# ubuntuslave/vo_single_camera_sos

Hardware: AMD Instinct MI355X
Metric: frame-pairs/sec (detect+match+triangulate+RANSAC) on 640x480 omni, 2000 kpts (higher is better)
Workload: dtype u8/f32/f64

## Files before the change

### vo_single_camera_sos_amd/csrc/ransac.hip

```cpp
#include <type_traits>
#include "common.h"
#include "ransac_core.h"
#include "epnp_core.h"
#include "gp3p_core.h"

namespace {

constexpr int kMaxCam = 8;
constexpr int kHypDoubles = 16;
constexpr int kThreads = 256;
constexpr int kScoreHypChunkMax = 128;

__device__ const double kEye9[9] = {1, 0, 0, 0, 1, 0, 0, 0, 1};
__device__ const double kZero3[3] = {0, 0, 0};

__device__ __forceinline__ uint64_t problem_seed(uint64_t seed, int b) { return seed + (uint64_t)b; }
__device__ __forceinline__ uint64_t problem_seed(const uint64_t* seeds, int b) { return seeds[b]; }

__global__ __launch_bounds__(kThreads) void ransac_prepare_kernel(const int32_t* __restrict__ cam,
                                                                  const int32_t* __restrict__ n_arr, int stride,
                                                                  int ncam, int32_t* __restrict__ perm,
                                                                  int32_t* __restrict__ cinfo,
                                                                  int32_t* __restrict__ split_out) {
  SOSVO_LATENCY_BOUND_PRIO();
// ... 137 lines not shown
                                                             const double* __restrict__ cam_off,
                                                             const double* __restrict__ cam_rot,
                                                             const int32_t* __restrict__ n_arr, int nprob, int stride,
                                                             int H, SeedT seed, double* __restrict__ hyp,
                                                             int32_t* __restrict__ counts) {
  SOSVO_LATENCY_BOUND_PRIO();
  int b, chunk;
  if (!hyp_block(nprob, (H + 63) >> 6, &b, &chunk)) return;
  const int it = chunk * 64 + threadIdx.x;
  const int n = min(n_arr[b], stride);
  const size_t base = (size_t)b * stride;
  const double* off = cam ? cam_off : kZero3;
  const double* rot = cam ? cam_rot : kEye9;
  double R[9], t[3];
  int ok = 0;
  if (it < H)
    ok = sv_hypothesis_gp3p(f + 3 * base, p + 3 * base, cam ? cam + base : nullptr, off, rot, n, problem_seed(seed, b),
                            (uint64_t)it, R, t);
  hyp_store_wave(hyp + (size_t)b * H * kHypDoubles, chunk * 64, H, ok != 0, R, t);
  if (it < H) counts[(size_t)b * H + it] = ok ? 0 : -1;
}

__device__ __forceinline__ int epnp_sample_front(const double* __restrict__ f, const double* __restrict__ p, int n, size_t base,
                                                 uint64_t seed, int it, double (&p6)[18], double (&uv)[2 * SV_EPNP_MAXN],
                                                 double (&cw)[12], double (&alphas)[4 * SV_EPNP_MAXN]) {
  int32_t s6[6];
  if (!sv_sample_distinct(n, 6, seed, (uint64_t)it, s6)) return 0;
  double f6[18];
#pragma unroll
  for (int k = 0; k < 6; ++k)
#pragma unroll
    for (int c = 0; c < 3; ++c) {
      f6[3 * k + c] = f[3 * (base + s6[k]) + c];
      p6[3 * k + c] = p[3 * (base + s6[k]) + c];
    }
  return sv_epnp_front(f6, p6, 6, uv, cw, alphas);
}

constexpr int kEpnpVecDoubles = 48;
template <class SeedT>
__global__ __launch_bounds__(64) void ransac_epnp_eigen_kernel(const double* __restrict__ f, const double* __restrict__ p,
                                                               const int32_t* __restrict__ n_arr, int nprob, int stride,
                                                               int H, SeedT seed, double* __restrict__ vvbuf,
                                                               int32_t* __restrict__ counts) {
  int b, chunk;
  if (!hyp_block(nprob, (H + 63) >> 6, &b, &chunk)) return;
  const int it = chunk * 64 + threadIdx.x;
  if (it >= H) return;
  const int n = min(n_arr[b], stride);
  double p6[18], uv[2 * SV_EPNP_MAXN], cw[12], alphas[4 * SV_EPNP_MAXN];
  int ok = epnp_sample_front(f, p, n, (size_t)b * stride, problem_seed(seed, b), it, p6, uv, cw, alphas);
  double* out = vvbuf + ((size_t)b * H + it) * kEpnpVecDoubles;
  if (ok) {
    double vv[48];
    ok = sv_epnp_null4_ql(alphas, uv, 6, vv);
    if (ok) {
#pragma unroll
      for (int k = 0; k < 48; ++k) out[k] = vv[k];
    }
  }
  counts[(size_t)b * H + it] = ok ? 0 : -1;
}

template <class SeedT>
__global__ __launch_bounds__(64) void ransac_epnp_pose_kernel(const double* __restrict__ f, const double* __restrict__ p,
                                                              const int32_t* __restrict__ n_arr, int nprob, int stride,
                                                              int H, SeedT seed, const double* __restrict__ vvbuf,
                                                              double* __restrict__ hyp, int32_t* __restrict__ counts) {
  SOSVO_LATENCY_BOUND_PRIO();
  int b, chunk;
  if (!hyp_block(nprob, (H + 63) >> 6, &b, &chunk)) return;
  const int it = chunk * 64 + threadIdx.x;
  const int n = min(n_arr[b], stride);
  double R[9], t[3];
  int ok = it < H && counts[(size_t)b * H + it] == 0;
  if (ok) {
    double p6[18], uv[2 * SV_EPNP_MAXN], cw[12], alphas[4 * SV_EPNP_MAXN], vv[48];
    ok = epnp_sample_front(f, p, n, (size_t)b * stride, problem_seed(seed, b), it, p6, uv, cw, alphas);
    const double* in = vvbuf + ((size_t)b * H + it) * kEpnpVecDoubles;
#pragma unroll
    for (int k = 0; k < 48; ++k) vv[k] = in[k];
    if (ok) ok = sv_epnp_back(p6, 6, uv, cw, alphas, vv, R, t);
  }
  hyp_store_wave(hyp + (size_t)b * H * kHypDoubles, chunk * 64, H, ok != 0, R, t);
  if (it < H) counts[(size_t)b * H + it] = ok ? 0 : -1;
}

template <bool IDENT>
__device__ __forceinline__ bool inlier_exact(const double* __restrict__ h, const double fx, const double fy,
                                             const double fz, const double px, const double py, const double pz,
                                             const double ox, const double oy, const double oz, const double* Rc,
                                             const double thr) {
  const double vx = (((h[0] * px) + (h[3] * py)) + (h[6] * pz)) + h[12];
  const double vy = (((h[1] * px) + (h[4] * py)) + (h[7] * pz)) + h[13];
  const double vz = (((h[2] * px) + (h[5] * py)) + (h[8] * pz)) + h[14];
  const double wx = vx - ox, wy = vy - oy, wz = vz - oz;
  double ux = wx, uy = wy, uz = wz;
  if (!IDENT) {
    ux = ((Rc[0] * wx) + (Rc[3] * wy)) + (Rc[6] * wz);
    uy = ((Rc[1] * wx) + (Rc[4] * wy)) + (Rc[7] * wz);
    uz = ((Rc[2] * wx) + (Rc[5] * wy)) + (Rc[8] * wz);
  }
  const double nrm = sqrt(((ux * ux) + (uy * uy)) + (uz * uz));
  const double gx = ux / nrm, gy = uy / nrm, gz = uz / nrm;
  return (1.0 - (((fx * gx) + (fy * gy)) + (fz * gz))) < thr;
}

constexpr double kTier1K = 1048576.0;
constexpr double kTier1Eps = 5.9604644775390625e-08;
constexpr double kTier1QBand = 3.47 / kTier1K + 20.0 * kTier1Eps;
constexpr double kTier1Max = 1e9;
constexpr double kTier1E2 = (3.47 * kTier1K + 6.0) * 78.03 * kTier1Eps * kTier1Eps * (1.0 + 1e-4);

__device__ __forceinline__ float score_tier1_lane(double fx, double fy, double fz, double px, double py, double pz, double ox,
                                                  double oy, double oz) {
  const double p1 = fabs(px) + fabs(py) + fabs(pz);
  const double om = fmax(fabs(ox), fmax(fabs(oy), fabs(oz)));
  const double fn = fx * fx + fy * fy + fz * fz;
  const double l = (p1 * p1 + om * om) * (1.0 + 1e-6);
  return (fabs(fn - 1.0) <= 1e-6 && p1 <= kTier1Max && om <= kTier1Max) ? (float)l : __builtin_inff();
}

__device__ __forceinline__ void score_tier1_hyp(const double* __restrict__ h, float* __restrict__ hs) {
  double rho = 0.0;
#pragma unroll
  for (int k = 0; k < 9; ++k) {
    hs[k] = (float)h[k];
    rho = fmax(rho, fabs(h[k]));
  }
  const double im = fmax(fabs(h[9]), fmax(fabs(h[10]), fabs(h[11])));
  hs[9] = (float)h[9], hs[10] = (float)h[10], hs[11] = (float)h[11];
  const double chk = (((((((h[0] + h[1]) + h[2]) + h[3]) + h[4]) + h[5]) + h[6]) + h[7]) + h[8] + h[9] + h[10] + h[11];
  const double ea = kTier1E2 * fmax(rho * rho, 1.0) * (1.0 + 1e-6);
  const double eb = kTier1E2 * (im * im) * (1.0 + 1e-6) + 1e-24;
  const bool fin = chk == chk && rho <= kTier1Max && im <= kTier1Max;
  hs[12] = fin ? (float)ea : __builtin_nanf("");
  hs[13] = fin ? (float)eb : __builtin_nanf("");
  hs[14] = 0.0f, hs[15] = 0.0f;
}

__device__ __forceinline__ int score_set_at(int E, int n, int split, int k) {
  if (split <= 0 || split >= n) return E - 1 - k;
  const int tb = split >> 6, nbot = E - 1 - tb, ntop = tb + 1, m = min(nbot, ntop);
  if (k < 2 * m) return (k & 1) ? tb - (k >> 1) : E - 1 - (k >> 1);
  return nbot > ntop ? E - 1 - (k - m) : tb - (k - m);
}

template <bool IDENT, int PPT, bool T1>
__global__ __launch_bounds__(kThreads) __attribute__((amdgpu_waves_per_eu(T1 ? 4 : 1))) void ransac_score_kernel(
    const double* __restrict__ f, const double* __restrict__ p, const int32_t* __restrict__ cam,
    const double* __restrict__ cam_off, const double* __restrict__ cam_rot, const int32_t* __restrict__ n_arr,
    int stride, int H, int hchunk, int hspan, double thr, int fast_ok, const double* __restrict__ hyp,
    int32_t* __restrict__ counts, int set_lo, int set_hi, int hsplit, const int32_t* __restrict__ alive_idx,
    const int32_t* __restrict__ n_alive, const int32_t* __restrict__ split_arr) {
  static_assert(!T1 || (IDENT && PPT <= 4), "tier 1 is written for the identity-rotation form");
  SOSVO_LATENCY_BOUND_PRIO();
  constexpr bool KEEP = !T1;
  __shared__ int lcnt[kScoreHypChunkMax];
  __shared__ double shyp[kScoreHypChunkMax][12];
  __shared__ unsigned long long sok[(kScoreHypChunkMax + 63) / 64];
  __shared__ int sidx[kScoreHypChunkMax];
  __shared__ int srec[kScoreHypChunkMax];
  __shared__ float shyp32[T1 ? kScoreHypChunkMax : 1][16];
  const int tid = threadIdx.x, b = blockIdx.z;
  const int n = min(n_arr[b], stride);
  const int Hb = alive_idx ? n_alive[b] : H;
  const int xspan = alive_idx ? (int)((blockIdx.x + blockIdx.z) % gridDim.x) : (int)blockIdx.x;
  if (xspan * hspan >= Hb) return;
  const int nset_all = (n + 63) >> 6, split = split_arr ? split_arr[b] : 0;
  auto set_at = [&](int k) { return split_arr ? score_set_at(nset_all, n, split, k) : k; };
  const int sbeg = set_lo, send = min(nset_all, set_hi);
  const int nsets = send - sbeg;
  const int bcap = hsplit ? PPT : (kThreads / 64) * PPT;
  const int nb = (nsets + bcap - 1) / bcap;
  if ((int)blockIdx.y >= nb) return;
  const int spb = (nsets + nb - 1) / nb;
  const int set0 = hsplit ? sbeg + ((int)blockIdx.y * nsets) / nb : sbeg + (int)blockIdx.y * spb;
  const int set1 = hsplit ? sbeg + (((int)blockIdx.y + 1) * nsets) / nb : min(set0 + spb, send);
  const int p0 = set_at(set0) * 64;

  double fx[KEEP ? PPT : 1], fy[KEEP ? PPT : 1], fz[KEEP ? PPT : 1];
  double px[KEEP ? PPT : 1], py[KEEP ? PPT : 1], pz[KEEP ? PPT : 1];
  double ox[KEEP ? PPT : 1], oy[KEEP ? PPT : 1], oz[KEEP ? PPT : 1];
  float fxs[T1 ? PPT : 1], fys[T1 ? PPT : 1], fzs[T1 ? PPT : 1], pxs[T1 ? PPT : 1], pys[T1 ? PPT : 1], pzs[T1 ? PPT : 1];
  float oxs[T1 ? PPT : 1], oys[T1 ? PPT : 1], ozs[T1 ? PPT : 1], lerr[T1 ? PPT : 1];
  int rowi[PPT];
  double Rc[IDENT ? 1 : 9];
  const int wave = __builtin_amdgcn_readfirstlane(tid >> 6), lane = tid & 63;
  const int wslot = (wave + blockIdx.x + blockIdx.y + blockIdx.z) & (kThreads / 64 - 1);
  const int jstep = hsplit ? kThreads / 64 : 1, jbeg = hsplit ? wslot : 0;
  const size_t base = (size_t)b * stride;
  unsigned long long vmask[PPT];
  int nlive_v = 0;
#pragma unroll
  for (int r = 0; r < PPT; ++r) {
    const int pos = set0 + (hsplit ? r : r * (kThreads / 64) + wslot);
    const int i0 = (pos < set1 ? set_at(pos) : nset_all) * 64;
    const int i = i0 + lane;
    nlive_v += pos < set1 ? 1 : 0;
    const bool valid = i < n;
    vmask[r] = __ballot(valid);
    rowi[r] = valid ? i : p0;
    const size_t row = base + rowi[r];
    const double lfx = f[3 * row + 0], lfy = f[3 * row + 1], lfz = f[3 * row + 2];
    const double lpx = p[3 * row + 0], lpy = p[3 * row + 1], lpz = p[3 * row + 2];
    const int c = cam ? cam[row] : 0;
    const double* o = cam ? cam_off + 3 * c : kZero3;
    const double lox = o[0], loy = o[1], loz = o[2];
    if (KEEP) {
      fx[r] = lfx, fy[r] = lfy, fz[r] = lfz;
      px[r] = lpx, py[r] = lpy, pz[r] = lpz;
      ox[r] = lox, oy[r] = loy, oz[r] = loz;
    }
    if (!IDENT) {
      const double* rc = cam ? cam_rot + 9 * c : kEye9;
#pragma unroll
      for (int k = 0; k < 9; ++k) Rc[k] = rc[k];
    }
    if (T1) {
      fxs[r] = (float)lfx, fys[r] = (float)lfy, fzs[r] = (float)lfz;
      pxs[r] = (float)lpx, pys[r] = (float)lpy, pzs[r] = (float)lpz;
      oxs[r] = (float)lox, oys[r] = (float)loy, ozs[r] = (float)loz;
      lerr[r] = score_tier1_lane(lfx, lfy, lfz, lpx, lpy, lpz, lox, loy, loz);
    }
  }
  const int nlive = __builtin_amdgcn_readfirstlane(nlive_v);
  const double c1 = 1.0 - thr;
  const double c2 = c1 * c1;
  const double c2hi = c2 * (1.0 + 1e-9), c2lo = c2 * (1.0 - 1e-9);
  const float c2hs = (float)((c2 + kTier1QBand) * (1.0 + 1e-6)), c2ls = (float)((c2 - kTier1QBand) * (1.0 - 1e-6));
  const int hend = min(Hb, (xspan + 1) * hspan);
  for (int h0 = xspan * hspan; h0 < hend; h0 += hchunk) {
  const int h1 = min(hend, h0 + hchunk);
  for (int k = tid; k < kScoreHypChunkMax; k += kThreads) lcnt[k] = 0;
  const int nh = h1 - h0;
  const double* hb = hyp + (size_t)b * H * kHypDoubles;
  static_assert(kScoreHypChunkMax == 128, "two words of solved-hypothesis flags");
  if (wave < 2) {
    const int hh = wave * 64 + lane;
    const int rec = hh < nh ? (alive_idx ? alive_idx[(size_t)b * H + h0 + hh] : h0 + hh) : 0;
    const double r00 = hh < nh ? hb[(size_t)rec * kHypDoubles] : 0.0;
    const unsigned long long okb = __ballot(hh < nh && r00 == r00);
    if (lane == 0) sok[wave] = okb;
    srec[hh] = rec;
  }
  __syncthreads();
  const unsigned long long ok0 = sok[0], ok1 = sok[1];
  const int nok = __builtin_amdgcn_readfirstlane(__popcll(ok0) + __popcll(ok1));
  for (int k = tid; k < nh * 12; k += kThreads) {
    const int hh = k / 12, e = k - hh * 12;
    const unsigned long long w = hh < 64 ? ok0 : ok1;
    if ((w >> (hh & 63)) & 1ULL) {
      const int pos = __popcll(w & ((1ULL << (hh & 63)) - 1ULL)) + (hh < 64 ? 0 : __popcll(ok0));
      const int rec = srec[hh];
      shyp[pos][e] = hb[(size_t)rec * kHypDoubles + (e < 9 ? e : e + 3)];
      if (e == 0) sidx[pos] = rec;
    }
  }
  __syncthreads();
  if (T1) {
    for (int pos = tid; pos < nok; pos += kThreads) score_tier1_hyp(shyp[pos], shyp32[pos]);
    __syncthreads();
  }

  auto tier2 = [&](auto nl, const int j, const unsigned long long* und1) -> int {
    constexpr int NL = decltype(nl)::value;
    int total = 0;
    const double* hp = shyp[j];
    const double r0 = hp[0], r1 = hp[1], r2 = hp[2], r3 = hp[3], r4 = hp[4], r5 = hp[5], r6 = hp[6], r7 = hp[7], r8 = hp[8];
    const double ix = hp[9], iy = hp[10], iz = hp[11];
#pragma unroll
    for (int r = 0; r < NL && r < PPT; ++r) {
      if (!und1[r]) continue;
      double Fx, Fy, Fz, Px, Py, Pz, Ox, Oy, Oz;
      if (KEEP) {
        Fx = fx[r], Fy = fy[r], Fz = fz[r], Px = px[r], Py = py[r], Pz = pz[r];
        Ox = ox[r], Oy = oy[r], Oz = oz[r];
      } else {
        const size_t row = base + rowi[r];
        Fx = f[3 * row + 0], Fy = f[3 * row + 1], Fz = f[3 * row + 2];
        Px = p[3 * row + 0], Py = p[3 * row + 1], Pz = p[3 * row + 2];
        const double* o = cam ? cam_off + 3 * cam[row] : kZero3;
        Ox = o[0], Oy = o[1], Oz = o[2];
      }
      unsigned long long und = und1[r];
      if (fast_ok) {
        double ux = fma(r0, Px, fma(r3, Py, fma(r6, Pz, ix - Ox)));
        double uy = fma(r1, Px, fma(r4, Py, fma(r7, Pz, iy - Oy)));
        double uz = fma(r2, Px, fma(r5, Py, fma(r8, Pz, iz - Oz)));
        if (!IDENT) {
          const double wx = ux, wy = uy, wz = uz;
          ux = fma(Rc[0], wx, fma(Rc[IDENT ? 0 : 3], wy, Rc[IDENT ? 0 : 6] * wz));
          uy = fma(Rc[IDENT ? 0 : 1], wx, fma(Rc[IDENT ? 0 : 4], wy, Rc[IDENT ? 0 : 7] * wz));
          uz = fma(Rc[IDENT ? 0 : 2], wx, fma(Rc[IDENT ? 0 : 5], wy, Rc[IDENT ? 0 : 8] * wz));
        }
        const double s = fma(Fx, ux, fma(Fy, uy, Fz * uz));
        const double q = fma(ux, ux, fma(uy, uy, uz * uz));
        const double lhs = s * s;
        const unsigned long long pos = __ballot(s > 0.0) & und1[r];
        const unsigned long long hi = __ballot(lhs > c2hi * q);
        const unsigned long long lo = __ballot(lhs < c2lo * q);
        total += __popcll(pos & hi);
        und = pos & ~hi & ~lo;
      }
      if (und) {
        const double vx = (((r0 * Px) + (r3 * Py)) + (r6 * Pz)) + ix;
        const double vy = (((r1 * Px) + (r4 * Py)) + (r7 * Pz)) + iy;
        const double vz = (((r2 * Px) + (r5 * Py)) + (r8 * Pz)) + iz;
        const double wx = vx - Ox, wy = vy - Oy, wz = vz - Oz;
        double ux = wx, uy = wy, uz = wz;
        if (!IDENT) {
          ux = ((Rc[0] * wx) + (Rc[IDENT ? 0 : 3] * wy)) + (Rc[IDENT ? 0 : 6] * wz);
          uy = ((Rc[IDENT ? 0 : 1] * wx) + (Rc[IDENT ? 0 : 4] * wy)) + (Rc[IDENT ? 0 : 7] * wz);
          uz = ((Rc[IDENT ? 0 : 2] * wx) + (Rc[IDENT ? 0 : 5] * wy)) + (Rc[IDENT ? 0 : 8] * wz);
        }
        const double q = ((ux * ux) + (uy * uy)) + (uz * uz);
        const double nrm = sqrt(q);
        const double gx = ux / nrm, gy = uy / nrm, gz = uz / nrm;
        total += __popcll(__ballot((1.0 - (((Fx * gx) + (Fy * gy)) + (Fz * gz))) < thr) & und);
      }
    }
    return total;
  };

  auto tier1 = [&](auto nl, const int j, unsigned long long* und1, unsigned long long& any1) -> int {
    constexpr int NL = decltype(nl)::value;
    int total = 0;
    const float* hs = shyp32[T1 ? j : 0];
    const float q0 = hs[0], q1 = hs[1], q2 = hs[2], q3 = hs[3], q4 = hs[4], q5 = hs[5], q6 = hs[6], q7 = hs[7], q8 = hs[8];
    const float jx = hs[9], jy = hs[10], jz = hs[11], ea = hs[12], eb = hs[13];
#pragma unroll
    for (int r = 0; r < NL && r < PPT; ++r) {
      const float ux = fmaf(q0, pxs[T1 ? r : 0], fmaf(q3, pys[T1 ? r : 0], fmaf(q6, pzs[T1 ? r : 0], jx - oxs[T1 ? r : 0])));
      const float uy = fmaf(q1, pxs[T1 ? r : 0], fmaf(q4, pys[T1 ? r : 0], fmaf(q7, pzs[T1 ? r : 0], jy - oys[T1 ? r : 0])));
      const float uz = fmaf(q2, pxs[T1 ? r : 0], fmaf(q5, pys[T1 ? r : 0], fmaf(q8, pzs[T1 ? r : 0], jz - ozs[T1 ? r : 0])));
      const float sv = fmaf(fxs[T1 ? r : 0], ux, fmaf(fys[T1 ? r : 0], uy, fzs[T1 ? r : 0] * uz));
      const float qv = fmaf(ux, ux, fmaf(uy, uy, uz * uz));
      const float lhs = sv * fabsf(sv);
      const float e2 = fmaf(ea, lerr[T1 ? r : 0], eb);
      const unsigned long long hi = __ballot(lhs > fmaf(c2hs, qv, e2));
      const unsigned long long lo = __ballot(lhs < fmaf(c2ls, qv, -e2));
      total += __popcll(hi & vmask[r]);
      und1[r] = ~hi & ~lo & vmask[r];
      any1 |= und1[r];
    }
    return total;
  };

  auto hyp_loop = [&](auto nl) {
    constexpr int NL = decltype(nl)::value;
    int cntv = 0, k = 0;
    for (int j = jbeg; j < nok; j += jstep, ++k) {
      unsigned long long und[PPT], any = 0ULL;
      int tot = 0;
      if (T1) {
        tot = tier1(nl, j, und, any);
      } else {
#pragma unroll
        for (int r = 0; r < NL && r < PPT; ++r) {
          und[r] = vmask[r];
          any |= vmask[r];
        }
      }
      if (any) tot += tier2(nl, j, und);
      if (lane == (k & 63)) cntv += tot;
      if ((k & 63) == 63) {
        if (cntv) atomicAdd(&lcnt[jbeg + ((k & ~63) + lane) * jstep], cntv);
        cntv = 0;
      }
    }
    if (cntv) atomicAdd(&lcnt[jbeg + (((k - 1) & ~63) + lane) * jstep], cntv);
  };
  if (nlive >= 4) hyp_loop(std::integral_constant<int, 4>{});
  else if (nlive == 3) hyp_loop(std::integral_constant<int, 3>{});
  else if (nlive == 2) hyp_loop(std::integral_constant<int, 2>{});
  else if (nlive == 1) hyp_loop(std::integral_constant<int, 1>{});
  __syncthreads();
  for (int k = tid; k < nok; k += kThreads) {
    const int v = lcnt[k];
    if (v) atomicAdd(&counts[(size_t)b * H + sidx[k]], v);
  }
  }
}

__global__ __launch_bounds__(kThreads) void ransac_prune_kernel(
    const double* __restrict__ f, const double* __restrict__ p, const int32_t* __restrict__ cam,
    const double* __restrict__ cam_off, const int32_t* __restrict__ n_arr, int stride, int H, int k_done, double thr,
    const double* __restrict__ hyp, const int32_t* __restrict__ counts, const int32_t* __restrict__ in_idx,
    const int32_t* __restrict__ n_in, int32_t* __restrict__ alive_idx, int32_t* __restrict__ n_alive,
    int32_t* __restrict__ state) {
  SOSVO_LATENCY_BOUND_PRIO();
  __shared__ long long red[kThreads / 64];
  __shared__ int redc[kThreads / 64];
  __shared__ int wave_off[kThreads / 64 + 1];
  const int tid = threadIdx.x, b = blockIdx.x, lane = tid & 63, wid = tid >> 6;
  const int n = min(n_arr[b], stride);
  const int32_t* cb = counts + (size_t)b * H;
  const int32_t* ib = in_idx ? in_idx + (size_t)b * H : nullptr;
  int32_t* ab = alive_idx + (size_t)b * H;
  const int Hin = in_idx ? n_in[b] : H;
  long long best_key = -1;
  for (int j = tid; j < Hin; j += kThreads) {
    const int it = ib ? ib[j] : j;
    const int c = cb[it];
    const long long key = ((long long)c << 32) | (long long)(0x7FFFFFFF - it);
    if (c >= 0 && key > best_key) best_key = key;
  }
  for (int o = 32; o > 0; o >>= 1) {
    const long long other = __shfl_down(best_key, o);
    best_key = other > best_key ? other : best_key;
  }
  if (lane == 0) red[wid] = best_key;
  __syncthreads();
  best_key = red[0];
  for (int w = 1; w < kThreads / 64; ++w) best_key = red[w] > best_key ? red[w] : best_key;
  if (best_key < 0) {
    if (tid == 0) n_alive[b] = 0;
    return;
  }
  const int hstar = 0x7FFFFFFF - (int)(best_key & 0xFFFFFFFFLL);
  const int L_prev = in_idx ? state[2 * b] : 0, h_prev = in_idx ? state[2 * b + 1] : -1;
  int L = L_prev;
  if (hstar != h_prev) {
    const double* hp = hyp + ((size_t)b * H + hstar) * kHypDoubles;
    const size_t base = (size_t)b * stride;
    int cnt = 0;
    for (int i = tid; i < n; i += kThreads) {
      const size_t row = base + i;
      const double* o = cam ? cam_off + 3 * cam[row] : kZero3;
      cnt += inlier_exact<true>(hp, f[3 * row], f[3 * row + 1], f[3 * row + 2], p[3 * row], p[3 * row + 1], p[3 * row + 2],
                                o[0], o[1], o[2], kEye9, thr) ? 1 : 0;
    }
    for (int o = 32; o > 0; o >>= 1) cnt += __shfl_down(cnt, o);
    if (lane == 0) redc[wid] = cnt;
    __syncthreads();
    L = max(L_prev, ((redc[0] + redc[1]) + redc[2]) + redc[3]);
  }
  const int rest = 64 * max(0, ((n + 63) >> 6) - k_done);
  int running = 0;
  for (int j0 = 0; j0 < Hin; j0 += kThreads) {
    const int j = j0 + tid;
    const int it = j < Hin ? (ib ? ib[j] : j) : 0;
    const int c = j < Hin ? cb[it] : -1;
    const bool keep = c >= 0 && c + rest >= L;
    const unsigned long long bal = __ballot(keep);
    __syncthreads();
    if (lane == 0) wave_off[wid + 1] = __popcll(bal);
    __syncthreads();
    int off = running;
    for (int w = 0; w < wid; ++w) off += wave_off[w + 1];
    if (keep) ab[off + __popcll(bal & ((1ULL << lane) - 1ULL))] = it;
    running += ((wave_off[1] + wave_off[2]) + wave_off[3]) + wave_off[4];
  }
  if (tid == 0) {
    n_alive[b] = running;
    state[2 * b] = L;
    state[2 * b + 1] = hstar;
  }
}

template <bool IDENT>
__global__ __launch_bounds__(kThreads) void ransac_select_kernel(
    const double* __restrict__ f, const double* __restrict__ p, const int32_t* __restrict__ cam,
    const double* __restrict__ cam_off, const double* __restrict__ cam_rot, const int32_t* __restrict__ n_arr,
    int stride, int H, double thr, int adaptive, const double* __restrict__ hyp, const int32_t* __restrict__ counts,
    double* __restrict__ T_out, uint8_t* __restrict__ mask, int32_t* __restrict__ inl_idx,
    int32_t* __restrict__ n_inl, int32_t* __restrict__ info) {
  SOSVO_LATENCY_BOUND_PRIO();
  __shared__ long long red[kThreads / 64];
  __shared__ int redv[kThreads / 64];
  __shared__ int s_best_it, s_used, s_nvalid;
  __shared__ int wave_off[kThreads / 64 + 1];
  __shared__ int s_running;
  const int tid = threadIdx.x, b = blockIdx.x, lane = tid & 63, wid = tid >> 6;
  const int n = min(n_arr[b], stride);
  const int32_t* cb = counts + (size_t)b * H;

  long long best_key = -1;
  int nvalid = 0;
  for (int it = tid; it < H; it += kThreads) {
    const int c = cb[it];
    if (c >= 0) {
      nvalid++;
      const long long key = ((long long)c << 32) | (long long)(0x7FFFFFFF - it);
      best_key = key > best_key ? key : best_key;
    }
  }
  for (int o = 32; o > 0; o >>= 1) {
    const long long other = __shfl_down(best_key, o);
    best_key = other > best_key ? other : best_key;
    nvalid += __shfl_down(nvalid, o);
  }
  if (lane == 0) {
    red[wid] = best_key;
    redv[wid] = nvalid;
  }
  __syncthreads();
  if (tid == 0) {
    long long k = red[0];
    int nv = redv[0];
    for (int w = 1; w < kThreads / 64; ++w) {
      k = red[w] > k ? red[w] : k;
      nv += redv[w];
    }
    s_nvalid = nv;
    if (!(adaptive & 1)) {
      s_best_it = k < 0 ? -1 : (0x7FFFFFFF - (int)(k & 0xFFFFFFFFLL));
      s_used = H;
    } else {
      int best_count = -1, best_it = -1, iterations = 0, used = 0;
      double base = 1.0;
      for (int it = 0; it < H; ++it) {
        if (iterations > 0 && !sv_ransac_continue(base, iterations)) break;
        used = it + 1;
        const int c = cb[it];
        if (c < 0) continue;
        if (c > best_count) {
          best_count = c;
          best_it = it;
          base = (adaptive & 2) ? sv_adaptive_base6(c, n) : ((adaptive & 4) ? sv_adaptive_base2(c, n) : sv_adaptive_base(c, n));
        }
        iterations++;
      }
      s_best_it = best_it;
      s_used = used;
    }
    s_running = 0;
  }
  __syncthreads();
  const int best_it = s_best_it;
  const size_t base = (size_t)b * stride;
  if (best_it < 0) {
    for (int i = tid; i < n; i += kThreads) mask[base + i] = 0;
// ... 161 lines not shown
        __syncthreads();
        continue;
      }
      if (s_flag == 4) {
        converged = 1;
        __syncthreads();
        break;
      }
      double xn[6];
#pragma unroll
      for (int u = 0; u < 6; ++u) xn[u] = sxn[u];
      double cn = 0.0;
      for (int q = tid; q < cnt; q += kThreads) {
        const int i = idx ? idx[base + q] : q;
        const size_t row = base + i;
        const int cc = cam ? cam[row] : 0;
        const double* o = cam ? cam_off + 3 * cc : kZero3;
        const double* rc = cam ? cam_rot + 9 * cc : kEye9;
        const double r = sv_residual(xn, f + 3 * row, p + 3 * row, o, rc);
        cn += r * r;
      }
      cn = block_sum(cn, scratch, tid);
      if (cn < cost) {
        converged = ((cost - cn) <= SV_LM_FTOL * cost);
        __syncthreads();
        if (tid == 0) {
#pragma unroll
          for (int u = 0; u < 6; ++u) sx[u] = xn[u];
        }
        cost = cn;
        lambda *= 0.1;
        if (lambda < 1e-15) lambda = 1e-15;
        accepted = 1;
        __syncthreads();
        break;
      }
      lambda *= 10.0;
      __syncthreads();
    }
    it_done = it + 1;
    if (!accepted || converged) break;
  }
  __syncthreads();
  if (tid == 0) {
    double R[9], t[3];
    sv_cayley2rot(sx + 3, R);
    t[0] = sx[0];
    t[1] = sx[1];
    t[2] = sx[2];
    sv_Rt_to_T(R, t, T);
    if (cost_out) cost_out[b] = cost;
    if (iters_out) iters_out[b] = it_done;
  }
}

}

template <class SeedT>
static int32_t ransac_abs_pose_impl(sosvo_ctx* ctx, const char* fn, const double* f, const double* p, const int32_t* cam,
                                    const double* cam_off, const double* cam_rot, int32_t ncam, int32_t flags,
                                    const int32_t* n, int32_t nprob, int32_t stride, double thr, int32_t max_iter,
                                    int32_t adaptive, SeedT seed, double* T_out,
                                    uint8_t* inlier_mask, int32_t* inlier_idx, int32_t* n_inliers, int32_t* info,
                                    int32_t* hyp_counts) {
#define SOSVO_LAUNCH_HYP(ctx, kernel, ...)              \
  do {                                                  \
    SOSVO_PROFILE(ctx, #kernel);                        \
    hipLaunchKernelGGL((kernel<SeedT>), __VA_ARGS__);   \
  } while (0)
#define SOSVO_REQUIRE_FN(ctx, cond, msg)                               \
  do {                                                                 \
    if (!(cond)) return sosvo_fail((ctx), SOSVO_ERR_ARG, fn, msg);     \
  } while (0)
  SOSVO_REQUIRE_FN(ctx, f && p && n && T_out && inlier_mask && inlier_idx && n_inliers && info, "null pointer");
  SOSVO_REQUIRE_FN(ctx, cam == nullptr || (cam_off && cam_rot), "cam given without cam_off / cam_rot");
  SOSVO_REQUIRE_FN(ctx, ncam >= 1 && ncam <= kMaxCam, "ncam out of range (1..8)");
  SOSVO_REQUIRE_FN(ctx, nprob >= 0 && nprob <= 65535, "nprob out of range");
  SOSVO_REQUIRE_FN(ctx, stride > 0 && stride <= (1 << 20), "stride out of range");
  SOSVO_REQUIRE_FN(ctx, max_iter > 0 && max_iter <= (1 << 20), "max_iter out of range");
  SOSVO_REQUIRE_FN(ctx, thr > 0.0, "threshold must be positive");
  if (nprob == 0) return SOSVO_OK;
  const int H = max_iter;
  size_t off = 0;
  auto carve = [&](size_t bytes) {
    size_t o = off;
    off += (bytes + 255) & ~(size_t)255;
    return o;
  };
  const size_t o_perm = carve(sizeof(int32_t) * (size_t)nprob * stride);
  const size_t o_cinfo = carve(sizeof(int32_t) * (size_t)nprob * (2 * kMaxCam + 1));
  const size_t o_hyp = carve(sizeof(double) * (size_t)nprob * H * kHypDoubles);
  const size_t o_counts = carve(sizeof(int32_t) * (size_t)nprob * H);
  const bool epnp_vec = (flags & SOSVO_FLAG_EPNP) != 0;
  const size_t o_vv = carve(epnp_vec ? sizeof(double) * (size_t)nprob * H * kEpnpVecDoubles : 0);
  const size_t o_alive = carve(sizeof(int32_t) * (size_t)nprob * (H + 1));
  const size_t o_alive2 = carve(sizeof(int32_t) * (size_t)nprob * (H + 1));
  const size_t o_stage = carve(sizeof(int32_t) * (size_t)nprob * 2);
  const size_t o_split = carve(sizeof(int32_t) * (size_t)nprob);
  int32_t rc = sosvo_ws_reserve(ctx, off);
  if (rc != SOSVO_OK) return rc;
  char* ws = (char*)ctx->ws;
  int32_t* perm = (int32_t*)(ws + o_perm);
  int32_t* cinfo = (int32_t*)(ws + o_cinfo);
  double* hyp = (double*)(ws + o_hyp);
  int32_t* counts = hyp_counts ? hyp_counts : (int32_t*)(ws + o_counts);
  int32_t* split = (int32_t*)(ws + o_split);

  SOSVO_LAUNCH(ctx,ransac_prepare_kernel, dim3(nprob), dim3(kThreads), 0, ctx->stream, cam, n, stride,
                     cam ? ncam : 1, perm, cinfo, split);
  SOSVO_LAUNCH_CHECK(ctx);
  const int epnp = (flags & SOSVO_FLAG_EPNP) != 0;
  SOSVO_REQUIRE_FN(ctx, !epnp || cam == nullptr, "SOSVO_FLAG_EPNP is for central problems (cam == NULL)");
  const int twopt = (flags & SOSVO_FLAG_TWOPT) != 0 && !epnp && !(flags & SOSVO_FLAG_GP3P);
  SOSVO_REQUIRE_FN(ctx, !twopt || cam == nullptr, "SOSVO_FLAG_TWOPT is for central problems (cam == NULL)");
  if (epnp) adaptive = (adaptive ? 1 : 0) | 2;
  if (twopt) adaptive = (adaptive ? 1 : 0) | 4;
  if (epnp) {
    double* vvbuf = (double*)(ws + o_vv);
    SOSVO_LAUNCH_HYP(ctx, ransac_epnp_eigen_kernel, dim3(hyp_grid(nprob, cdiv(H, 64))), dim3(64), 0, ctx->stream, f, p, n, nprob, stride, H,
                 seed, vvbuf, counts);
    SOSVO_LAUNCH_HYP(ctx, ransac_epnp_pose_kernel, dim3(hyp_grid(nprob, cdiv(H, 64))), dim3(64), 0, ctx->stream, f, p, n, nprob, stride, H,
                 seed, vvbuf, hyp, counts);
  } else if (twopt) {
    SOSVO_LAUNCH_HYP(ctx, ransac_hyp_twopt_kernel, dim3(hyp_grid(nprob, cdiv(H, 64))), dim3(64), 0, ctx->stream, f, p, n, nprob, stride, H, seed,
                 hyp, counts);
  } else if (flags & SOSVO_FLAG_GP3P) {
    SOSVO_LAUNCH_HYP(ctx, ransac_hyp_gp3p_kernel, dim3(hyp_grid(nprob, cdiv(H, 64))), dim3(64), 0, ctx->stream, f, p, cam, cam_off, cam_rot,
                 n, nprob, stride, H, seed, hyp, counts);
  } else
    SOSVO_LAUNCH_HYP(ctx, ransac_hyp_kernel, dim3(hyp_grid(nprob, cdiv(H, 64))), dim3(64), 0, ctx->stream, f, p, cam, cam_off, cam_rot, n,
                 nprob, stride, H, seed, perm, cinfo, hyp, counts);
  SOSVO_LAUNCH_CHECK(ctx);

  const bool ident = (flags & SOSVO_FLAG_CAM_ROT_IDENTITY) != 0 || cam == nullptr;
  const int fast_ok = thr < 0.5 ? 1 : 0;
  const int ppt = ident ? 4 : 1;
  const int gx = cdiv(stride, kThreads * ppt);
  const bool t1 = ident && fast_ok && !ctx->hint_score_fp64_only;
  const int wg_target = t1 ? 4096 : 8192;
  int hchunks = cdiv(wg_target, nprob);
  if (hchunks < 1) hchunks = 1;
  int hspan = cdiv(H, hchunks);
  if (hspan < 32) hspan = H < 32 ? H : 32;
  hchunks = cdiv(H, hspan);
  const int hchunk = cdiv(hspan, cdiv(hspan, kScoreHypChunkMax));
  dim3 grid(hchunks, gx, nprob);
  constexpr int kProbeSets = 4, kPruneMinSets = 8, kStageMinSets = 16, kPruneMinProblems = 64;
#ifndef SOSVO_STAGE_PLAN
#define SOSVO_STAGE_PLAN 4, 14
#endif
  static const int kStagePlan[] = {SOSVO_STAGE_PLAN};
  const bool prune = t1 && adaptive == 0 && hyp_counts == nullptr && !epnp && !twopt && stride >= 64 * kPruneMinSets &&
                     nprob >= kPruneMinProblems;
#define SOSVO_SCORE_ARGS grid, dim3(kThreads), 0, ctx->stream, f, p, cam, cam_off, cam_rot, n, stride, H, hchunk, hspan, thr, fast_ok, hyp, counts, 0, INT_MAX, 0, (const int32_t*)nullptr, (const int32_t*)nullptr, (const int32_t*)nullptr
  if (prune) {
    const int capsets = cdiv(stride, 64);
    const bool staged = stride >= 64 * kStageMinSets;
    int nstage = 1;
    if (staged)
      for (nstage = 0; nstage < (int)(sizeof(kStagePlan) / sizeof(kStagePlan[0])) && kStagePlan[nstage] < capsets;) ++nstage;
    int32_t* alive_idx[2] = {(int32_t*)(ws + o_alive), (int32_t*)(ws + o_alive2)};
    int32_t* stage_state = (int32_t*)(ws + o_stage);
    auto pass = [&](int k_lo, int k_hi, const int32_t* list) {
      const int sets = min(k_hi, capsets) - k_lo;
      int hs = min(H, (sets <= 4 ? 4 : 2) * hspan);
      if (list) hs = min(H, max(kScoreHypChunkMax, hs));
      const int hck = cdiv(hs, cdiv(hs, kScoreHypChunkMax));
      SOSVO_LAUNCH(ctx,(ransac_score_kernel<true, 4, true>), dim3(cdiv(H, hs), cdiv(sets, 4), nprob), dim3(kThreads), 0,
                   ctx->stream, f, p, cam, cam_off, cam_rot, n, stride, H, hck, hs, thr, fast_ok, hyp, counts, k_lo, k_hi, 1,
                   list, list ? list + (size_t)nprob * H : nullptr, split);
    };
    int k_lo = 0;
    const int32_t* list = nullptr;
    for (int s = 0; s < nstage; ++s) {
      const int k_hi = staged ? kStagePlan[s] : kProbeSets;
      pass(k_lo, k_hi, list);
      int32_t* out = alive_idx[s & 1];
      SOSVO_LAUNCH(ctx,ransac_prune_kernel, dim3(nprob), dim3(kThreads), 0, ctx->stream, f, p, cam, cam_off, n, stride, H,
                   k_hi, thr, hyp, counts, list, list ? list + (size_t)nprob * H : nullptr, out, out + (size_t)nprob * H,
                   stage_state);
      list = out;
      k_lo = k_hi;
    }
    pass(k_lo, INT_MAX, list);
  } else if (t1)
    SOSVO_LAUNCH(ctx,(ransac_score_kernel<true, 4, true>), SOSVO_SCORE_ARGS);
  else if (ident)
    SOSVO_LAUNCH(ctx,(ransac_score_kernel<true, 4, false>), SOSVO_SCORE_ARGS);
  else
    SOSVO_LAUNCH(ctx,(ransac_score_kernel<false, 1, false>), SOSVO_SCORE_ARGS);
#undef SOSVO_SCORE_ARGS
  SOSVO_LAUNCH_CHECK(ctx);
  if (ident)
    SOSVO_LAUNCH(ctx,(ransac_select_kernel<true>), dim3(nprob), dim3(kThreads), 0, ctx->stream, f, p, cam,
                       cam_off, cam_rot, n, stride, H, thr, adaptive, hyp, counts, T_out, inlier_mask, inlier_idx,
                       n_inliers, info);
  else
    SOSVO_LAUNCH(ctx,(ransac_select_kernel<false>), dim3(nprob), dim3(kThreads), 0, ctx->stream, f, p, cam,
                       cam_off, cam_rot, n, stride, H, thr, adaptive, hyp, counts, T_out, inlier_mask, inlier_idx,
                       n_inliers, info);
  SOSVO_LAUNCH_CHECK(ctx);
  return SOSVO_OK;
}
#undef SOSVO_REQUIRE_FN
#undef SOSVO_LAUNCH_HYP

extern "C" {

int32_t sosvo_ransac_abs_pose(sosvo_ctx* ctx, const double* f, const double* p, const int32_t* cam,
                              const double* cam_off, const double* cam_rot, int32_t ncam, int32_t flags,
                              const int32_t* n, int32_t nprob, int32_t stride, double thr, int32_t max_iter,
                              int32_t adaptive, uint64_t seed, double* T_out, uint8_t* inlier_mask,
                              int32_t* inlier_idx, int32_t* n_inliers, int32_t* info, int32_t* hyp_counts) {
  SOSVO_ENTER(ctx);
  return ransac_abs_pose_impl(ctx, __func__, f, p, cam, cam_off, cam_rot, ncam, flags, n, nprob, stride, thr, max_iter, adaptive,
                              seed, T_out, inlier_mask, inlier_idx, n_inliers, info, hyp_counts);
}

int32_t sosvo_ransac_abs_pose_seeds(sosvo_ctx* ctx, const double* f, const double* p, const int32_t* cam,
                                    const double* cam_off, const double* cam_rot, int32_t ncam, int32_t flags,
                                    const int32_t* n, int32_t nprob, int32_t stride, double thr, int32_t max_iter,
                                    int32_t adaptive, const uint64_t* seeds, double* T_out, uint8_t* inlier_mask,
                                    int32_t* inlier_idx, int32_t* n_inliers, int32_t* info, int32_t* hyp_counts) {
  SOSVO_ENTER(ctx);
  SOSVO_REQUIRE(ctx, seeds, "null seed array");
  return ransac_abs_pose_impl(ctx, __func__, f, p, cam, cam_off, cam_rot, ncam, flags, n, nprob, stride, thr, max_iter, adaptive,
                              seeds, T_out, inlier_mask, inlier_idx, n_inliers, info, hyp_counts);
}

int32_t sosvo_refine_abs_pose(sosvo_ctx* ctx, const double* f, const double* p, const int32_t* cam,
                              const double* cam_off, const double* cam_rot, int32_t ncam, const int32_t* n,
                              int32_t nprob, int32_t stride, const int32_t* idx, const int32_t* m,
                              int32_t max_lm_iter, double* T_io, double* cost_out, int32_t* iters_out) {
  SOSVO_ENTER(ctx);
  SOSVO_REQUIRE(ctx, f && p && n && T_io, "null pointer");
  SOSVO_REQUIRE(ctx, cam == nullptr || (cam_off && cam_rot), "cam given without cam_off / cam_rot");
  SOSVO_REQUIRE(ctx, (idx == nullptr) == (m == nullptr), "idx and m go together");
  SOSVO_REQUIRE(ctx, ncam >= 1 && ncam <= kMaxCam, "ncam out of range (1..8)");
  SOSVO_REQUIRE(ctx, nprob >= 0 && nprob <= 65535, "nprob out of range");
  SOSVO_REQUIRE(ctx, stride > 0 && stride <= (1 << 20), "stride out of range");
  SOSVO_REQUIRE(ctx, max_lm_iter > 0 && max_lm_iter <= 10000, "max_lm_iter out of range");
  if (nprob == 0) return SOSVO_OK;
  SOSVO_LAUNCH(ctx,refine_kernel, dim3(nprob), dim3(kThreads), 0, ctx->stream, f, p, cam, cam_off, cam_rot, n,
                     stride, idx, m, max_lm_iter, T_io, cost_out, iters_out);
  SOSVO_LAUNCH_CHECK(ctx);
  return SOSVO_OK;
}

}
```

Baseline: 72210.

## Walk remaining point sets in-block with per-hypothesis early termination in pruned scoring

In the pruned-list scoring passes, each block now walks every remaining point-set group itself instead of spreading them across grid.y. It keeps running inlier counts per hypothesis in shared memory and drops a hypothesis once its count plus the remaining points cannot reach the stage threshold. Survivors are compacted in shared memory, so later groups score fewer hypotheses, and the block exits when none remain. This trades grid-level parallelism over point sets for skipped work, and it replaces atomics with direct stores because each hypothesis chunk is owned by a single block.

```diff
diff --git a/vo_single_camera_sos_amd/csrc/ransac.hip b/vo_single_camera_sos_amd/csrc/ransac.hip
--- a/vo_single_camera_sos_amd/csrc/ransac.hip
+++ b/vo_single_camera_sos_amd/csrc/ransac.hip
@@ -313,7 +313,7 @@
     const double* __restrict__ cam_off, const double* __restrict__ cam_rot, const int32_t* __restrict__ n_arr,
     int stride, int H, int hchunk, int hspan, double thr, int fast_ok, const double* __restrict__ hyp,
     int32_t* __restrict__ counts, int set_lo, int set_hi, int hsplit, const int32_t* __restrict__ alive_idx,
-    const int32_t* __restrict__ n_alive, const int32_t* __restrict__ split_arr) {
+    const int32_t* __restrict__ n_alive, const int32_t* __restrict__ split_arr, const int32_t* __restrict__ stage_state) {
   static_assert(!T1 || (IDENT && PPT <= 4), "tier 1 is written for the identity-rotation form");
   SOSVO_LATENCY_BOUND_PRIO();
   constexpr bool KEEP = !T1;
@@ -323,8 +323,10 @@
   __shared__ int sidx[kScoreHypChunkMax];
   __shared__ int srec[kScoreHypChunkMax];
   __shared__ float shyp32[T1 ? kScoreHypChunkMax : 1][16];
+  __shared__ int sbase[T1 ? kScoreHypChunkMax : 1];
   const int tid = threadIdx.x, b = blockIdx.z;
   const int n = min(n_arr[b], stride);
+  const bool walk = T1 && alive_idx != nullptr;
   const int Hb = alive_idx ? n_alive[b] : H;
   const int xspan = alive_idx ? (int)((blockIdx.x + blockIdx.z) % gridDim.x) : (int)blockIdx.x;
   if (xspan * hspan >= Hb) return;
@@ -334,11 +336,11 @@
   const int nsets = send - sbeg;
   const int bcap = hsplit ? PPT : (kThreads / 64) * PPT;
   const int nb = (nsets + bcap - 1) / bcap;
-  if ((int)blockIdx.y >= nb) return;
+  const int yb0 = walk ? 0 : (int)blockIdx.y, yb1 = walk ? nb : yb0 + 1;
+  if (yb0 >= nb) return;
   const int spb = (nsets + nb - 1) / nb;
-  const int set0 = hsplit ? sbeg + ((int)blockIdx.y * nsets) / nb : sbeg + (int)blockIdx.y * spb;
-  const int set1 = hsplit ? sbeg + (((int)blockIdx.y + 1) * nsets) / nb : min(set0 + spb, send);
-  const int p0 = set_at(set0) * 64;
+  const int Lb = walk ? stage_state[2 * b] : 0;
+  int nok = 0;
 
   double fx[KEEP ? PPT : 1], fy[KEEP ? PPT : 1], fz[KEEP ? PPT : 1];
   double px[KEEP ? PPT : 1], py[KEEP ? PPT : 1], pz[KEEP ? PPT : 1];
@@ -348,10 +350,20 @@
   int rowi[PPT];
   double Rc[IDENT ? 1 : 9];
   const int wave = __builtin_amdgcn_readfirstlane(tid >> 6), lane = tid & 63;
-  const int wslot = (wave + blockIdx.x + blockIdx.y + blockIdx.z) & (kThreads / 64 - 1);
-  const int jstep = hsplit ? kThreads / 64 : 1, jbeg = hsplit ? wslot : 0;
+  const int wrot = wave + blockIdx.x + blockIdx.z;
+  const int jstep = hsplit ? kThreads / 64 : 1;
   const size_t base = (size_t)b * stride;
   unsigned long long vmask[PPT];
+  const double c1 = 1.0 - thr;
+  const double c2 = c1 * c1;
+  const double c2hi = c2 * (1.0 + 1e-9), c2lo = c2 * (1.0 - 1e-9);
+  const float c2hs = (float)((c2 + kTier1QBand) * (1.0 + 1e-6)), c2ls = (float)((c2 - kTier1QBand) * (1.0 - 1e-6));
+  for (int yb = yb0; yb < yb1; ++yb) {
+  const int set0 = hsplit ? sbeg + (yb * nsets) / nb : sbeg + yb * spb;
+  const int set1 = hsplit ? sbeg + ((yb + 1) * nsets) / nb : min(set0 + spb, send);
+  const int p0 = set_at(set0) * 64;
+  const int wslot = (wrot + yb) & (kThreads / 64 - 1);
+  const int jbeg = hsplit ? wslot : 0;
   int nlive_v = 0;
 #pragma unroll
   for (int r = 0; r < PPT; ++r) {
@@ -386,42 +398,45 @@
     }
   }
   const int nlive = __builtin_amdgcn_readfirstlane(nlive_v);
-  const double c1 = 1.0 - thr;
-  const double c2 = c1 * c1;
-  const double c2hi = c2 * (1.0 + 1e-9), c2lo = c2 * (1.0 - 1e-9);
-  const float c2hs = (float)((c2 + kTier1QBand) * (1.0 + 1e-6)), c2ls = (float)((c2 - kTier1QBand) * (1.0 - 1e-6));
   const int hend = min(Hb, (xspan + 1) * hspan);
   for (int h0 = xspan * hspan; h0 < hend; h0 += hchunk) {
   const int h1 = min(hend, h0 + hchunk);
-  for (int k = tid; k < kScoreHypChunkMax; k += kThreads) lcnt[k] = 0;
   const int nh = h1 - h0;
   const double* hb = hyp + (size_t)b * H * kHypDoubles;
-  static_assert(kScoreHypChunkMax == 128, "two words of solved-hypothesis flags");
+  static_assert(kScoreHypChunkMax == 128 && kThreads == 2 * kScoreHypChunkMax, "two words of flags, two threads an entry");
+  if (!walk || yb == 0) {
+  int ts = tid;
+  asm volatile("" : "+v"(ts));
+  for (int k = ts; k < kScoreHypChunkMax; k += kThreads) lcnt[k] = 0;
   if (wave < 2) {
-    const int hh = wave * 64 + lane;
+    const int hh = ts;
     const int rec = hh < nh ? (alive_idx ? alive_idx[(size_t)b * H + h0 + hh] : h0 + hh) : 0;
     const double r00 = hh < nh ? hb[(size_t)rec * kHypDoubles] : 0.0;
     const unsigned long long okb = __ballot(hh < nh && r00 == r00);
-    if (lane == 0) sok[wave] = okb;
+    if ((ts & 63) == 0) sok[wave] = okb;
     srec[hh] = rec;
   }
   __syncthreads();
   const unsigned long long ok0 = sok[0], ok1 = sok[1];
-  const int nok = __builtin_amdgcn_readfirstlane(__popcll(ok0) + __popcll(ok1));
-  for (int k = tid; k < nh * 12; k += kThreads) {
+  nok = __builtin_amdgcn_readfirstlane(__popcll(ok0) + __popcll(ok1));
+  for (int k = ts; k < nh * 12; k += kThreads) {
     const int hh = k / 12, e = k - hh * 12;
     const unsigned long long w = hh < 64 ? ok0 : ok1;
     if ((w >> (hh & 63)) & 1ULL) {
       const int pos = __popcll(w & ((1ULL << (hh & 63)) - 1ULL)) + (hh < 64 ? 0 : __popcll(ok0));
       const int rec = srec[hh];
       shyp[pos][e] = hb[(size_t)rec * kHypDoubles + (e < 9 ? e : e + 3)];
-      if (e == 0) sidx[pos] = rec;
+      if (e == 0) {
+        sidx[pos] = rec;
+        if (walk) sbase[T1 ? pos : 0] = counts[(size_t)b * H + rec];
+      }
     }
   }
   __syncthreads();
   if (T1) {
-    for (int pos = tid; pos < nok; pos += kThreads) score_tier1_hyp(shyp[pos], shyp32[pos]);
+    for (int pos = ts; pos < nok; pos += kThreads) score_tier1_hyp(shyp[pos], shyp32[pos]);
     __syncthreads();
+  }
   }
 
   auto tier2 = [&](auto nl, const int j, const unsigned long long* und1) -> int {
@@ -438,7 +453,9 @@
         Fx = fx[r], Fy = fy[r], Fz = fz[r], Px = px[r], Py = py[r], Pz = pz[r];
         Ox = ox[r], Oy = oy[r], Oz = oz[r];
       } else {
-        const size_t row = base + rowi[r];
+        int ri = rowi[r];
+        asm volatile("" : "+v"(ri));
+        const size_t row = base + ri;
         Fx = f[3 * row + 0], Fy = f[3 * row + 1], Fz = f[3 * row + 2];
         Px = p[3 * row + 0], Py = p[3 * row + 1], Pz = p[3 * row + 2];
         const double* o = cam ? cam_off + 3 * cam[row] : kZero3;
@@ -537,9 +554,64 @@
   else if (nlive == 2) hyp_loop(std::integral_constant<int, 2>{});
   else if (nlive == 1) hyp_loop(std::integral_constant<int, 1>{});
   __syncthreads();
-  for (int k = tid; k < nok; k += kThreads) {
-    const int v = lcnt[k];
-    if (v) atomicAdd(&counts[(size_t)b * H + sidx[k]], v);
+  if (!walk) {
+    for (int k = tid; k < nok; k += kThreads) {
+      const int v = lcnt[k];
+      if (v) atomicAdd(&counts[(size_t)b * H + sidx[k]], v);
+    }
+  } else if constexpr (T1) {
+    const bool lastb = yb + 1 == yb1;
+    const int rest = 64 * (nset_all - set1);
+    int t = tid;
+    asm volatile("" : "+v"(t));
+    const int tl = t & 63;
+    int run = 0, rec = 0;
+    bool keep = false;
+    if (wave < 2) {
+      const bool valid = t < nok;
+      const int add = lcnt[t];
+      run = sbase[t] + add, rec = sidx[t];
+      keep = valid && !lastb && run + rest >= Lb;
+      if (valid && !keep) counts[(size_t)b * H + rec] = run;
+      const unsigned long long kb = __ballot(keep);
+      if (tl == 0) sok[wave] = kb;
+      lcnt[t] = 0;
+    }
+    if (!lastb) {
+      __syncthreads();
+      const unsigned long long kw0 = sok[0], kw1 = sok[1];
+      const int nkeep = __builtin_amdgcn_readfirstlane(__popcll(kw0) + __popcll(kw1));
+      if (nkeep == 0) return;
+      if (nkeep == nok) {
+        if (wave < 2) sbase[t] = run;
+      } else {
+        const int e = t >> 1, half = t & 1;
+        const unsigned long long w = e < 64 ? kw0 : kw1;
+        const bool mine = (w >> (e & 63)) & 1ULL;
+        const int to = __popcll(w & ((1ULL << (e & 63)) - 1ULL)) + (e < 64 ? 0 : __popcll(kw0));
+        double md[6];
+        float ms[8];
+#pragma unroll
+        for (int i = 0; i < 6; ++i) md[i] = shyp[e][6 * half + i];
+#pragma unroll
+        for (int i = 0; i < 8; ++i) ms[i] = shyp32[T1 ? e : 0][8 * half + i];
+        __syncthreads();
+        if (mine) {
+#pragma unroll
+          for (int i = 0; i < 6; ++i) shyp[to][6 * half + i] = md[i];
+#pragma unroll
+          for (int i = 0; i < 8; ++i) shyp32[T1 ? to : 0][8 * half + i] = ms[i];
+        }
+        if (keep) {
+          const int pos = __popcll((wave ? kw1 : kw0) & ((1ULL << tl) - 1ULL)) + (wave ? __popcll(kw0) : 0);
+          sbase[pos] = run;
+          sidx[pos] = rec;
+        }
+        nok = nkeep;
+      }
+      __syncthreads();
+    }
+  }
   }
   }
 }
@@ -1007,7 +1079,7 @@
   static const int kStagePlan[] = {SOSVO_STAGE_PLAN};
   const bool prune = t1 && adaptive == 0 && hyp_counts == nullptr && !epnp && !twopt && stride >= 64 * kPruneMinSets &&
                      nprob >= kPruneMinProblems;
-#define SOSVO_SCORE_ARGS grid, dim3(kThreads), 0, ctx->stream, f, p, cam, cam_off, cam_rot, n, stride, H, hchunk, hspan, thr, fast_ok, hyp, counts, 0, INT_MAX, 0, (const int32_t*)nullptr, (const int32_t*)nullptr, (const int32_t*)nullptr
+#define SOSVO_SCORE_ARGS grid, dim3(kThreads), 0, ctx->stream, f, p, cam, cam_off, cam_rot, n, stride, H, hchunk, hspan, thr, fast_ok, hyp, counts, 0, INT_MAX, 0, (const int32_t*)nullptr, (const int32_t*)nullptr, (const int32_t*)nullptr, (const int32_t*)nullptr
   if (prune) {
     const int capsets = cdiv(stride, 64);
     const bool staged = stride >= 64 * kStageMinSets;
@@ -1019,11 +1091,11 @@
     auto pass = [&](int k_lo, int k_hi, const int32_t* list) {
       const int sets = min(k_hi, capsets) - k_lo;
       int hs = min(H, (sets <= 4 ? 4 : 2) * hspan);
-      if (list) hs = min(H, max(kScoreHypChunkMax, hs));
+      if (list) hs = min(H, kScoreHypChunkMax);
       const int hck = cdiv(hs, cdiv(hs, kScoreHypChunkMax));
-      SOSVO_LAUNCH(ctx,(ransac_score_kernel<true, 4, true>), dim3(cdiv(H, hs), cdiv(sets, 4), nprob), dim3(kThreads), 0,
+      SOSVO_LAUNCH(ctx,(ransac_score_kernel<true, 4, true>), dim3(cdiv(H, hs), list ? 1 : cdiv(sets, 4), nprob), dim3(kThreads), 0,
                    ctx->stream, f, p, cam, cam_off, cam_rot, n, stride, H, hck, hs, thr, fast_ok, hyp, counts, k_lo, k_hi, 1,
-                   list, list ? list + (size_t)nprob * H : nullptr, split);
+                   list, list ? list + (size_t)nprob * H : nullptr, split, stage_state);
     };
     int k_lo = 0;
     const int32_t* list = nullptr;
```

New measurement: 72380, median of 6. Within noise of the previous version (+0.2%).
